# roeiherz/CanonicalSg2Im

Hardware: NVIDIA B200
Metric: scene_graphs_per_sec_gcn_layout_fwd_bwd (higher is better)
Workload: dtype bf16

## Files before the change

### canonicalsg2im_b200/csrc/gemm_tc.cu

```cuda
#include "common.cuh"
#include "internal.h"
#include <cuda.h>
#include <cuda_bf16.h>
#include <cuda_fp16.h>
#include <stdlib.h>
#include <string.h>

namespace {

constexpr int BLOCK_M = 128;
constexpr int BLOCK_K = 64;
constexpr int MAX_STAGES = 8;
constexpr int A_STAGE_BYTES = BLOCK_M * BLOCK_K * 2;
constexpr int GATHER_WARPS = 4;
constexpr int ACC_STRIDE = 256;
constexpr int SUB_N = 32;
constexpr int SUB_BYTES = 32 * SUB_N * 2;
constexpr int CHUNK_N = 64;
constexpr int CHUNK_BYTES = 32 * CHUNK_N * 2;
constexpr size_t SMEM_LIMIT = 232448;

enum { G_NONE = 0, G_A = 1, G_B = 2 };

struct TcParams {
  int M, N, K;
  int m_tiles, n_tiles, splits, kb_per_split, kb_total;
  int stages;
  int smem_epi;
  void* C;
  int ldc, out_f32;
  const float* bias;
  int relu;
  const float* rowscale;
  const __nv_bfloat16* mask_aux;
  int ld_aux;
  const int* g_sidx;
  const int* g_oidx;
  const int* g_pidx;
  int g_din, g_dp, g_rows;
  int debug;
  int a_f16, b_f16, c_f16;
  int tail_from, num_items;
};

__device__ __forceinline__ uint32_t smem_u32(const void* p) { return (uint32_t)__cvta_generic_to_shared(p); }

__device__ __forceinline__ void mbar_init(uint32_t bar, uint32_t count) {
  asm volatile("mbarrier.init.shared::cta.b64 [%0], %1;" ::"r"(bar), "r"(count));
}
__device__ __forceinline__ void mbar_arrive_expect_tx(uint32_t bar, uint32_t bytes) {
  asm volatile("mbarrier.arrive.expect_tx.shared::cta.b64 _, [%0], %1;" ::"r"(bar), "r"(bytes) : "memory");
}
// ... 115 lines not shown
      "%16, %17, %18, %19, %20, %21, %22, %23, %24, %25, %26, %27, %28, %29, %30, %31}, [%32];"
      : "=r"(r[0]), "=r"(r[1]), "=r"(r[2]), "=r"(r[3]), "=r"(r[4]), "=r"(r[5]), "=r"(r[6]), "=r"(r[7]),
        "=r"(r[8]), "=r"(r[9]), "=r"(r[10]), "=r"(r[11]), "=r"(r[12]), "=r"(r[13]), "=r"(r[14]), "=r"(r[15]),
        "=r"(r[16]), "=r"(r[17]), "=r"(r[18]), "=r"(r[19]), "=r"(r[20]), "=r"(r[21]), "=r"(r[22]), "=r"(r[23]),
        "=r"(r[24]), "=r"(r[25]), "=r"(r[26]), "=r"(r[27]), "=r"(r[28]), "=r"(r[29]), "=r"(r[30]), "=r"(r[31])
      : "r"(taddr)
      : "memory");
}
__device__ __forceinline__ void tmem_ld_wait() { asm volatile("tcgen05.wait::ld.sync.aligned;" ::: "memory"); }

__device__ __forceinline__ uint64_t make_desc(uint32_t saddr, uint32_t lbo_bytes, uint32_t sbo_bytes) {
  uint64_t d = 0;
  d |= (uint64_t)((saddr & 0x3FFFFu) >> 4);
  d |= (uint64_t)((lbo_bytes >> 4) & 0x3FFFu) << 16;
  d |= (uint64_t)((sbo_bytes >> 4) & 0x3FFFu) << 32;
  d |= (uint64_t)1 << 46;
  d |= (uint64_t)2 << 61;
  return d;
}
__host__ __device__ constexpr uint32_t make_idesc(int M, int N, bool a_mn, bool b_mn, bool a_f16 = false, bool b_f16 = false) {
  return (1u << 4) | ((a_f16 ? 0u : 1u) << 7) | ((b_f16 ? 0u : 1u) << 10) | ((a_mn ? 1u : 0u) << 15) |
         ((b_mn ? 1u : 0u) << 16) | ((uint32_t)(N >> 3) << 17) | ((uint32_t)(M >> 4) << 24);
}

struct __align__(8) Barriers {
  uint64_t full[MAX_STAGES];
  uint64_t empty[MAX_STAGES];
  uint64_t tmem_full[2];
  uint64_t tmem_empty[2];
  uint32_t tmem_base;
};

struct SmemPlan {
  uint32_t b, c, bias, bars, total;
};
__host__ __device__ inline SmemPlan smem_plan(int BN, int b_rows, int stages, bool smem_epi, int mt, int epw, bool sub32) {
  SmemPlan s;
  (void)BN;
  s.b = (uint32_t)stages * mt * A_STAGE_BYTES;
  s.c = s.b + (uint32_t)stages * b_rows * 128;
  s.bias = s.c + (smem_epi ? epw * (sub32 ? SUB_BYTES : CHUNK_BYTES) : 0);
  s.bars = s.bias + (smem_epi ? epw * (sub32 ? SUB_N : CHUNK_N) * 4 : 0);
  s.total = s.bars + (uint32_t)sizeof(Barriers);
  return s;
}

__device__ __forceinline__ uint32_t pack_bf16(float a, float b) {
  __nv_bfloat162 h = __floats2bfloat162_rn(a, b);
  return *reinterpret_cast<uint32_t*>(&h);
}
__device__ __forceinline__ uint32_t pack16(float a, float b, bool f16) {
  if (!f16) return pack_bf16(a, b);
  __half2 h = __floats2half2_rn(fminf(fmaxf(a, -65504.f), 65504.f), fminf(fmaxf(b, -65504.f), 65504.f));
  return *reinterpret_cast<uint32_t*>(&h);
}
__device__ __forceinline__ bool bf16_pos(uint32_t h) { return h != 0 && h < 0x8000u; }

template <int BN, bool MN, int GATHER, int CG, int MT, int EPW, bool SUB32>
__global__ void __launch_bounds__(64 + EPW * 32 + (GATHER != G_NONE ? GATHER_WARPS * 32 : 0), 1)
gemm_tc_kernel(const __grid_constant__ CUtensorMap tmA, const __grid_constant__ CUtensorMap tmB,
               const __grid_constant__ CUtensorMap tmP, const TcParams p) {
  extern __shared__ __align__(1024) uint8_t smem_raw[];
  const uint32_t base = smem_u32(smem_raw);
  uint8_t* base_ptr = smem_raw;
  if ((base & 1023u) != 0u) {
    if (threadIdx.x == 0) printf("csg gemm_tc: dynamic shared memory is not 1024-byte aligned\n");
    __trap();
  }
  static_assert(CG == 1 || !MN, "CTA pairs are implemented for the K-major kernels");
  static_assert(MT == 1 || (MN && GATHER == G_B && CG == 1 && MT * BN <= 512), "MT > 1: gathered-B MN-major kernels only");
  static_assert(EPW == 8 || EPW == 16, "epilogue warps: 2 or 4 per TMEM lane quarter");
  constexpr int EPI_WARPS = EPW;
  constexpr int FIRST_GATHER_WARP = 2 + EPW;
  constexpr int NSUB = EPW / 4;
  constexpr int A_STAGE = MT * A_STAGE_BYTES;
  constexpr int B_ROWS = BN / CG;
  constexpr int B_STAGE = B_ROWS * BLOCK_K * 2;
  constexpr int TILE_M = BLOCK_M * CG * MT;
  const uint32_t cta_rank = CG == 2 ? cluster_ctarank() : 0u;
  const int worker = CG == 2 ? (int)(blockIdx.x >> 1) : (int)blockIdx.x;
  const int nworkers = CG == 2 ? (int)(gridDim.x >> 1) : (int)gridDim.x;
  const bool has_aux = GATHER == G_NONE && p.mask_aux != nullptr;
  const SmemPlan plan = smem_plan(BN, B_ROWS, p.stages, p.smem_epi != 0, MT, EPW, SUB32);
  const uint32_t sA = base, sB = base + plan.b;
  Barriers* bars = reinterpret_cast<Barriers*>(base_ptr + plan.bars);
  const int warp = threadIdx.x >> 5, lane = threadIdx.x & 31;
  const int num_tiles = p.num_items;
  const int STAGES = p.stages;

  if (warp == 1 && lane == 0) {
    for (int s = 0; s < STAGES; ++s) {
      mbar_init(smem_u32(&bars->full[s]), 1);
      mbar_init(smem_u32(&bars->empty[s]), 1);
    }
    for (int s = 0; s < 2; ++s) {
      mbar_init(smem_u32(&bars->tmem_full[s]), 1);
      mbar_init(smem_u32(&bars->tmem_empty[s]), EPI_WARPS * CG);
    }
    asm volatile("fence.mbarrier_init.release.cluster;" ::: "memory");
  }
  if (warp == 0 && lane == 0) {
    tma_prefetch_desc(&tmA);
    tma_prefetch_desc(&tmB);
    if (GATHER != G_NONE) tma_prefetch_desc(&tmP);
  }
  if (warp == 2) {
    if (CG == 2) { tmem_alloc_pair(smem_u32(&bars->tmem_base), 512); tmem_relinquish_pair(); }
    else { tmem_alloc(smem_u32(&bars->tmem_base), 512); tmem_relinquish(); }
  }
  tc_fence_before();
  if (CG == 2) cluster_sync_all(); else __syncthreads();
  tc_fence_after();
  asm volatile("griddepcontrol.wait;" ::: "memory");
  const uint32_t tmem_base = bars->tmem_base;
  auto leader = [&](const uint64_t* bar) -> uint32_t { return CG == 2 ? mapa(smem_u32(bar), 0u) : smem_u32(bar); };

// ... 174 lines not shown
              uint64_t ad, bd;
              if (!MN) {
                ad = make_desc(a_base + k * 32, 16, 1024);
                bd = make_desc(b_base + k * 32, 16, 1024);
              } else {
                ad = make_desc(a_base + mi * A_STAGE_BYTES + k * 2048, 8192, 1024);
                bd = make_desc(b_base + k * 2048, 8192, 1024);
              }
              if (p.debug & 2) continue;
              if (CG == 2) umma_bf16_pair(d_tmem, ad, bd, idesc, (kb > kb0 || k > 0) ? 1u : 0u);
              else umma_bf16(d_tmem + mi * BN, ad, bd, idesc, (kb > kb0 || k > 0) ? 1u : 0u);
            }
          }
          if (CG == 2) {
            umma_commit_pair(smem_u32(&bars->empty[stage]));
            if (kb == kb1 - 1) umma_commit_pair(smem_u32(&bars->tmem_full[as]));
          } else {
            umma_commit(smem_u32(&bars->empty[stage]));
            if (kb == kb1 - 1) umma_commit(smem_u32(&bars->tmem_full[as]));
          }
          if (++stage == STAGES) { stage = 0; phase ^= 1; }
        }
        if (kb1 <= kb0) {
          if (CG == 2) umma_commit_pair(smem_u32(&bars->tmem_full[as])); else umma_commit(smem_u32(&bars->tmem_full[as]));
        }
      }
    }
  } else if (warp < FIRST_GATHER_WARP) {
    const int q = warp & 3;
    const int ew = warp - 2;
    const int sub = ew >> 2;
    int it = 0;
    if (!MN && p.smem_epi) {
      if constexpr (SUB32) {
      const uint32_t sC = base + plan.c + ew * SUB_BYTES;
      float* sbias = reinterpret_cast<float*>(base_ptr + plan.bias) + ew * SUB_N;
      const uint32_t sw = ((uint32_t)lane >> 1) & 3u;
      const uint32_t row_off = (uint32_t)lane * (SUB_N * 2);
      const int crow = lane >> 2, cpiece = lane & 3;
      __nv_bfloat16* Cb = reinterpret_cast<__nv_bfloat16*>(p.C);
      const bool cf16 = p.c_f16 != 0;
      for (int tile = worker; tile < num_tiles; tile += nworkers, ++it) {
        int mt, nt, sp, n0, nw;
        decode(tile, mt, nt, sp, n0, nw);
        const int as = it & 1, aphase = (it >> 1) & 1;
        const int row0 = mt * TILE_M + (int)cta_rank * BLOCK_M + q * 32;
        const int row = row0 + lane;
        const int ncols = min(nw, p.N - n0);
        const int nsb = (ncols + SUB_N - 1) / SUB_N;
        const bool warp_rows = row0 < p.M;
        const float rs = (p.rowscale && row < p.M) ? __ldg(p.rowscale + row) : 1.f;
        mbar_wait(smem_u32(&bars->tmem_full[as]), aphase);
        tc_fence_after();
        const uint32_t t_row = tmem_base + ((uint32_t)(q * 32) << 16) + as * ACC_STRIDE;
        const int my_last = nsb > sub ? ((nsb - 1 - sub) / NSUB) * NSUB + sub : -1;
        if ((p.debug & 4) || my_last < 0) {
          tc_fence_before();
          __syncwarp();
          if (lane == 0) { if (CG == 2) mbar_arrive_cluster(leader(&bars->tmem_empty[as])); else mbar_arrive(smem_u32(&bars->tmem_empty[as])); }
          continue;
        }
#pragma unroll 1
        for (int c = sub; c < nsb; c += NSUB) {
          const int col0 = n0 + c * SUB_N;
          const float bv = p.bias ? __ldg(p.bias + col0 + lane) : 0.f;
          uint32_t r[32];
          tmem_ld32(t_row + c * SUB_N, r);
          const int col = col0 + cpiece * 8;
          uint4 ax[4];
          if (has_aux && warp_rows) {
#pragma unroll
            for (int i = 0; i < 4; ++i) {
              const int rr = row0 + i * 8 + crow;
              ax[i] = rr < p.M ? __ldg(reinterpret_cast<const uint4*>(p.mask_aux + (size_t)rr * p.ld_aux + col))
                               : make_uint4(0u, 0u, 0u, 0u);
            }
          }
          tmem_ld_wait();
          if (c == my_last) {
            tc_fence_before();
            __syncwarp();
            if (lane == 0) { if (CG == 2) mbar_arrive_cluster(leader(&bars->tmem_empty[as])); else mbar_arrive(smem_u32(&bars->tmem_empty[as])); }
          }
          if (warp_rows) {
            float v[32];
#pragma unroll
            for (int j = 0; j < 32; ++j) v[j] = __uint_as_float(r[j]);
            if (p.bias) {
              sbias[lane] = bv;
              __syncwarp();
#pragma unroll
              for (int j = 0; j < 32; j += 4) {
                const float4 b = *reinterpret_cast<const float4*>(sbias + j);
                v[j] += b.x; v[j + 1] += b.y; v[j + 2] += b.z; v[j + 3] += b.w;
              }
            }
            if (p.relu) {
#pragma unroll
              for (int j = 0; j < 32; ++j) v[j] = fmaxf(v[j], 0.f);
            }
            if (p.rowscale) {
#pragma unroll
              for (int j = 0; j < 32; ++j) v[j] *= rs;
            }
#pragma unroll
            for (int j4 = 0; j4 < 4; ++j4) {
              const uint32_t off = row_off + ((((uint32_t)j4) ^ sw) << 4);
              const uint32_t u0 = pack16(v[j4 * 8], v[j4 * 8 + 1], cf16), u1 = pack16(v[j4 * 8 + 2], v[j4 * 8 + 3], cf16);
              const uint32_t u2 = pack16(v[j4 * 8 + 4], v[j4 * 8 + 5], cf16), u3 = pack16(v[j4 * 8 + 6], v[j4 * 8 + 7], cf16);
              asm volatile("st.shared.v4.u32 [%0], {%1, %2, %3, %4};" ::"r"(sC + off), "r"(u0), "r"(u1), "r"(u2), "r"(u3) : "memory");
            }
            __syncwarp();
#pragma unroll
            for (int i = 0; i < 4; ++i) {
              const int rl = i * 8 + crow;
              uint4 o;
              asm volatile("ld.shared.v4.u32 {%0, %1, %2, %3}, [%4];" : "=r"(o.x), "=r"(o.y), "=r"(o.z), "=r"(o.w)
                           : "r"(sC + (uint32_t)rl * (SUB_N * 2) + ((uint32_t)(cpiece ^ ((rl >> 1) & 3)) << 4)));
              if (has_aux) {
                const uint32_t a[4] = {ax[i].x, ax[i].y, ax[i].z, ax[i].w};
                uint32_t w[4] = {o.x, o.y, o.z, o.w};
#pragma unroll
                for (int e = 0; e < 4; ++e) {
                  if (!bf16_pos(a[e] & 0xFFFFu)) w[e] &= 0xFFFF0000u;
                  if (!bf16_pos(a[e] >> 16)) w[e] &= 0x0000FFFFu;
                }
                o = make_uint4(w[0], w[1], w[2], w[3]);
              }
              if (row0 + rl < p.M)
                *reinterpret_cast<uint4*>(Cb + (size_t)(row0 + rl) * p.ldc + col) = o;
            }
            __syncwarp();
          }
        }
      }
      } else {
      const uint32_t sC = base + plan.c + ew * CHUNK_BYTES;
      float* sbias = reinterpret_cast<float*>(base_ptr + plan.bias) + ew * CHUNK_N;
      const uint32_t sw = (uint32_t)(lane & 7) << 4;
      const uint32_t row_off = (uint32_t)lane * 128;
      const int crow = lane >> 3, cpiece = lane & 7;
      __nv_bfloat16* Cb = reinterpret_cast<__nv_bfloat16*>(p.C);
      const bool cf16 = p.c_f16 != 0;
      auto load_mask = [&](uint4 (&ax)[8], int row0, int col) {
#pragma unroll
        for (int i = 0; i < 8; ++i) {
          const int r = row0 + i * 4 + crow;
          ax[i] = (r < p.M && col < p.N) ? __ldg(reinterpret_cast<const uint4*>(p.mask_aux + (size_t)r * p.ld_aux + col))
                                         : make_uint4(0u, 0u, 0u, 0u);
        }
      };
      for (int tile = worker; tile < num_tiles; tile += nworkers, ++it) {
        int mt, nt, sp, n0, nw;
        decode(tile, mt, nt, sp, n0, nw);
        const int as = it & 1, aphase = (it >> 1) & 1;
        const int row0 = mt * TILE_M + (int)cta_rank * BLOCK_M + q * 32;
        const int row = row0 + lane;
        const int ncols = min(nw, p.N - n0);
        const int nchunks = (ncols + CHUNK_N - 1) / CHUNK_N;
        const bool warp_rows = row0 < p.M;
        const float rs = (p.rowscale && row < p.M) ? __ldg(p.rowscale + row) : 1.f;
        mbar_wait(smem_u32(&bars->tmem_full[as]), aphase);
        tc_fence_after();
        const uint32_t t_row = tmem_base + ((uint32_t)(q * 32) << 16) + as * ACC_STRIDE;
        const int my_last = nchunks > sub ? ((nchunks - 1 - sub) / NSUB) * NSUB + sub : -1;
        if ((p.debug & 4) || my_last < 0) {
          tc_fence_before();
          __syncwarp();
          if (lane == 0) { if (CG == 2) mbar_arrive_cluster(leader(&bars->tmem_empty[as])); else mbar_arrive(smem_u32(&bars->tmem_empty[as])); }
          continue;
        }
#pragma unroll 1
        for (int c = sub; c < nchunks; c += NSUB) {
          const int bc = n0 + c * CHUNK_N + lane;
          const float bv0 = (p.bias && bc < p.N) ? __ldg(p.bias + bc) : 0.f;
          const float bv1 = (p.bias && bc + 32 < p.N) ? __ldg(p.bias + bc + 32) : 0.f;
          uint32_t r0[32], r1[32];
          tmem_ld32(t_row + c * CHUNK_N, r0);
          tmem_ld32(t_row + c * CHUNK_N + 32, r1);
          const int col = n0 + c * CHUNK_N + cpiece * 8;
          uint4 ax[8];
          if (has_aux && warp_rows) load_mask(ax, row0, col);
          tmem_ld_wait();
          if (c == my_last) {
            tc_fence_before();
            __syncwarp();
            if (lane == 0) { if (CG == 2) mbar_arrive_cluster(leader(&bars->tmem_empty[as])); else mbar_arrive(smem_u32(&bars->tmem_empty[as])); }
          }
          if (warp_rows) {
            if (p.bias) {
              sbias[lane] = bv0; sbias[lane + 32] = bv1;
              __syncwarp();
            }
#pragma unroll
            for (int h = 0; h < 2; ++h) {
              float v[32];
#pragma unroll
              for (int j = 0; j < 32; ++j) v[j] = __uint_as_float(h ? r1[j] : r0[j]);
              if (p.bias) {
#pragma unroll
                for (int j = 0; j < 32; j += 4) {
                  float4 b = *reinterpret_cast<const float4*>(sbias + h * 32 + j);
                  v[j] += b.x; v[j + 1] += b.y; v[j + 2] += b.z; v[j + 3] += b.w;
                }
              }
              if (p.relu) {
#pragma unroll
                for (int j = 0; j < 32; ++j) v[j] = fmaxf(v[j], 0.f);
              }
              if (p.rowscale) {
#pragma unroll
                for (int j = 0; j < 32; ++j) v[j] *= rs;
              }
#pragma unroll
              for (int j4 = 0; j4 < 4; ++j4) {
                const uint32_t off = row_off + ((((uint32_t)(h * 4 + j4)) << 4) ^ sw);
                const uint32_t u0 = pack16(v[j4 * 8], v[j4 * 8 + 1], cf16), u1 = pack16(v[j4 * 8 + 2], v[j4 * 8 + 3], cf16);
                const uint32_t u2 = pack16(v[j4 * 8 + 4], v[j4 * 8 + 5], cf16), u3 = pack16(v[j4 * 8 + 6], v[j4 * 8 + 7], cf16);
                asm volatile("st.shared.v4.u32 [%0], {%1, %2, %3, %4};" ::"r"(sC + off), "r"(u0), "r"(u1), "r"(u2), "r"(u3) : "memory");
              }
            }
            __syncwarp();
#pragma unroll
            for (int i = 0; i < 8; ++i) {
              const int rl = i * 4 + crow;
              uint4 o;
              asm volatile("ld.shared.v4.u32 {%0, %1, %2, %3}, [%4];" : "=r"(o.x), "=r"(o.y), "=r"(o.z), "=r"(o.w)
                           : "r"(sC + (uint32_t)rl * 128 + ((uint32_t)(cpiece ^ (rl & 7)) << 4)));
              if (has_aux) {
                const uint32_t a[4] = {ax[i].x, ax[i].y, ax[i].z, ax[i].w};
                uint32_t w[4] = {o.x, o.y, o.z, o.w};
#pragma unroll
                for (int e = 0; e < 4; ++e) {
                  if (!bf16_pos(a[e] & 0xFFFFu)) w[e] &= 0xFFFF0000u;
                  if (!bf16_pos(a[e] >> 16)) w[e] &= 0x0000FFFFu;
                }
                o = make_uint4(w[0], w[1], w[2], w[3]);
              }
              if (row0 + rl < p.M && col < p.N)
                *reinterpret_cast<uint4*>(Cb + (size_t)(row0 + rl) * p.ldc + col) = o;
            }
            __syncwarp();
          }
        }
      }
      }
    } else {
      for (int tile = worker; tile < num_tiles; tile += nworkers, ++it) {
        int mt, nt, sp, n0, nw;
        decode(tile, mt, nt, sp, n0, nw);
        const int as = it & 1, aphase = (it >> 1) & 1;
        mbar_wait(smem_u32(&bars->tmem_full[as]), aphase);
        tc_fence_after();
#pragma unroll 1
        for (int ci = sub; ci < MT * (BN / 32); ci += NSUB) {
          const int mi = ci / (BN / 32), c = ci % (BN / 32);
          const int row = mt * TILE_M + (int)cta_rank * BLOCK_M + mi * BLOCK_M + q * 32 + lane;
          const bool rowok = row < p.M;
          const float rs = (p.rowscale && rowok) ? p.rowscale[row] : 1.f;
          const uint32_t t_row = tmem_base + ((uint32_t)(q * 32) << 16) + as * ACC_STRIDE + mi * BN;
          uint32_t r[32];
          tmem_ld32(t_row + c * 32, r);
          tmem_ld_wait();
          const int col = nt * BN + c * 32;
          if (rowok && col < p.N) {
            float v[32];
#pragma unroll
            for (int j = 0; j < 32; ++j) v[j] = __uint_as_float(r[j]);
            if (p.splits == 1) {
              if (p.bias) {
#pragma unroll
                for (int j = 0; j < 32; j += 4) {
                  float4 b = __ldg(reinterpret_cast<const float4*>(p.bias + col + j));
                  v[j] += b.x; v[j + 1] += b.y; v[j + 2] += b.z; v[j + 3] += b.w;
                }
              }
              if (p.relu) {
#pragma unroll
// ... 52 lines not shown

EncodeTiledFn get_encode() {
  static EncodeTiledFn fn = nullptr;
  if (!fn) {
    void* ptr = nullptr;
    cudaDriverEntryPointQueryResult q;
    if (cudaGetDriverEntryPoint("cuTensorMapEncodeTiled", &ptr, cudaEnableDefault, &q) == cudaSuccess &&
        q == cudaDriverEntryPointSuccess)
      fn = reinterpret_cast<EncodeTiledFn>(ptr);
  }
  return fn;
}

int make_map(CUtensorMap* map, const void* ptr, uint64_t inner, uint64_t outer, uint64_t row_bytes, uint32_t box_outer) {
  EncodeTiledFn enc = get_encode();
  CSG_REQUIRE(enc != nullptr, "gemm_tc: cuTensorMapEncodeTiled is not available from the driver");
  CSG_REQUIRE((reinterpret_cast<uintptr_t>(ptr) & 15) == 0 && (row_bytes & 15) == 0,
              "gemm_tc: operand pointer / pitch must be 16-byte aligned");
  cuuint64_t dims[2] = {inner, outer};
  cuuint64_t strides[1] = {row_bytes};
  cuuint32_t box[2] = {64, box_outer};
  cuuint32_t estr[2] = {1, 1};
  CUresult r = enc(map, CU_TENSOR_MAP_DATA_TYPE_BFLOAT16, 2, const_cast<void*>(ptr), dims, strides, box, estr,
                   CU_TENSOR_MAP_INTERLEAVE_NONE, CU_TENSOR_MAP_SWIZZLE_128B, CU_TENSOR_MAP_L2_PROMOTION_L2_256B,
                   CU_TENSOR_MAP_FLOAT_OOB_FILL_NONE);
  CSG_REQUIRE(r == CUDA_SUCCESS, "gemm_tc: cuTensorMapEncodeTiled failed (%d)", (int)r);
  return 0;
}

struct Maps {
  CUtensorMap a, b, p;
};

template <int BN, bool MN, int GATHER, int CG, int MT = 1, int EPW = 8, bool SUB32 = false>
int launch(const Maps& m, const TcParams& p, cudaStream_t stream) {
  const size_t smem = smem_plan(BN, BN / CG, p.stages, p.smem_epi != 0, MT, EPW, SUB32).total;
  CSG_REQUIRE(smem <= SMEM_LIMIT, "gemm_tc: shared-memory plan of %zu bytes exceeds the limit", smem);
  static bool configured = false;
  if (!configured) {
    CSG_CUDA(cudaFuncSetAttribute(gemm_tc_kernel<BN, MN, GATHER, CG, MT, EPW, SUB32>, cudaFuncAttributeMaxDynamicSharedMemorySize, (int)SMEM_LIMIT));
    configured = true;
  }
  const int tiles = p.m_tiles * p.n_tiles * p.splits;
  const int nthreads = 64 + EPW * 32 + (GATHER != G_NONE ? GATHER_WARPS * 32 : 0);
  if (CG == 1) {
    const int grid = tiles < csg_num_sms() ? tiles : csg_num_sms();
    cudaLaunchConfig_t cfg;
    memset(&cfg, 0, sizeof(cfg));
    cfg.gridDim = dim3(grid);
    cfg.blockDim = dim3(nthreads);
    cfg.dynamicSmemBytes = smem;
    cfg.stream = stream;
    cudaLaunchAttribute attr[1];
    attr[0].id = cudaLaunchAttributeProgrammaticStreamSerialization;
    attr[0].val.programmaticStreamSerializationAllowed = 1;
    cfg.attrs = attr; cfg.numAttrs = 1;
    CSG_CUDA(cudaLaunchKernelEx(&cfg, gemm_tc_kernel<BN, MN, GATHER, CG, MT, EPW, SUB32>, m.a, m.b, m.p, p));
  } else {
    const int pairs = csg_num_sms() / 2;
    cudaLaunchConfig_t cfg;
    memset(&cfg, 0, sizeof(cfg));
    cfg.gridDim = dim3(2 * (tiles < pairs ? tiles : pairs));
    cfg.blockDim = dim3(nthreads);
    cfg.dynamicSmemBytes = smem;
    cfg.stream = stream;
    cudaLaunchAttribute attr[2];
    attr[0].id = cudaLaunchAttributeClusterDimension;
    attr[0].val.clusterDim.x = 2; attr[0].val.clusterDim.y = 1; attr[0].val.clusterDim.z = 1;
    attr[1].id = cudaLaunchAttributeProgrammaticStreamSerialization;
    attr[1].val.programmaticStreamSerializationAllowed = 1;
    cfg.attrs = attr; cfg.numAttrs = 2;
    CSG_CUDA(cudaLaunchKernelEx(&cfg, gemm_tc_kernel<BN, MN, GATHER, CG, MT, EPW, SUB32>, m.a, m.b, m.p, p));
  }
  CSG_CHECK_LAUNCH("csg_gemm_bf16");
  return 0;
}

template <bool MN, int GATHER, int CG, int EPW = 8, bool SUB32 = false>
int launch_bn(int BN, const Maps& m, const TcParams& p, cudaStream_t stream) {
  switch (BN) {
    case 64: return launch<64, MN, GATHER, CG, 1, EPW, SUB32>(m, p, stream);
    case 128: return launch<128, MN, GATHER, CG, 1, EPW, SUB32>(m, p, stream);
    case 192: return launch<192, MN, GATHER, CG, 1, EPW, SUB32>(m, p, stream);
    case 256: return launch<256, MN, GATHER, CG, 1, EPW, SUB32>(m, p, stream);
  }
  csg_set_error("gemm_tc: unsupported BLOCK_N %d", BN);
  return 1;
}

int g_pair_mode = -1;

int kmajor_pick_bn(int M, int N) {
  int bn = N > 128 ? 256 : (N > 64 ? 128 : 64);
  const int m_tiles = csg_div_up(M, BLOCK_M);
  while (bn > 64 && m_tiles * csg_div_up(N, bn) < csg_num_sms()) bn >>= 1;
  return bn;
}

int pick_bn(int N) {
  if (N % 256 == 0) return 256;
  if (N % 192 == 0) return 192;
  if (N % 128 == 0) return 128;
  if (N >= 256) return 256;
  if (N > 128) return 192 >= N ? 192 : 256;
  if (N > 64) return 128;
  return 64;
}

void mn_split_plan(int M, int N, int K, int BN, int& kb_per_split, int& nsplits, int mt = 1) {
  const int tiles = csg_div_up(M, BLOCK_M * mt) * csg_div_up(N, BN);
  const int kb_total = csg_div_up(K, BLOCK_K);
  int splits = csg_num_sms() / tiles;
  if (splits < 1) splits = 1;
  if (splits > 64) splits = 64;
  if (splits > kb_total) splits = kb_total;
  kb_per_split = csg_div_up(kb_total, splits);
  nsplits = csg_div_up(kb_total, kb_per_split);
// ... 35 lines not shown
                                      mask_aux, ld_aux, g_obj, g_pred, g_sidx, g_oidx, g_din, g_dp, g_ldp, g_nobj, g_pidx, g_npred,
                                      formats, workspace, workspace_bytes, stream, &job)) return rc;
  return job.parts > 0 ? csg_reduce_multi(&job, 1, stream) : 0;
}

int csg_gemm_bf16_deferred(int mn_major, int gather, int M, int N, int K,
                           const void* A, int lda, const void* B, int ldb, void* C, int ldc, int out_f32,
                           const float* bias, int relu, const float* rowscale, const void* mask_aux, int ld_aux,
                           const void* g_obj, const void* g_pred, const int* g_sidx, const int* g_oidx,
                           int g_din, int g_dp, int g_ldp, int g_nobj, const int* g_pidx, int g_npred, int formats,
                           void* workspace, size_t workspace_bytes, cudaStream_t stream, CsgReduceJob* job) {
  job->parts = 0; job->n = 0; job->partial = nullptr; job->out = nullptr; job->stride = 0; job->lanes = 1;
  job->op = CSG_RED_SUM; job->aux = nullptr; job->ncols = 0; job->ldo = 0;
  if (M == 0 || N == 0) return 0;
  if (K == 0 && mn_major && out_f32 && M > 0 && N > 0) {
    CSG_CUDA(cudaMemset2DAsync(C, (size_t)ldc * 4, 0, (size_t)N * 4, M, stream));
    return 0;
  }
  CSG_REQUIRE(M > 0 && N > 0 && K > 0, "gemm_bf16: bad sizes M=%d N=%d K=%d", M, N, K);
  CsgProfScope prof(CSG_PROF_GEMM_BF16, 2.0 * M * N * K, stream);
  CSG_REQUIRE(N % 32 == 0, "gemm_bf16: N=%d must be a multiple of 32", N);
  CSG_REQUIRE((ldc % 8) == 0 || out_f32, "gemm_bf16: bf16 ldc must be a multiple of 8");
  CSG_REQUIRE(!out_f32 || (ldc % 4) == 0, "gemm_bf16: fp32 ldc must be a multiple of 4");
  TcParams p;
  p.M = M; p.N = N; p.K = K;
  p.C = C; p.ldc = ldc; p.out_f32 = out_f32;
  p.bias = bias; p.relu = relu; p.rowscale = rowscale;
  p.mask_aux = reinterpret_cast<const __nv_bfloat16*>(mask_aux); p.ld_aux = ld_aux;
  p.g_sidx = g_sidx; p.g_oidx = g_oidx; p.g_din = g_din; p.g_dp = g_dp;
  p.g_pidx = gather ? g_pidx : nullptr;
  CSG_REQUIRE(!p.g_pidx || g_npred > 0, "gemm_bf16: g_pidx needs the row count of the predicate table");
  p.g_rows = mn_major ? K : M;
  p.a_f16 = formats & 1; p.b_f16 = (formats >> 1) & 1; p.c_f16 = (formats >> 2) & 1;
  { const char* dbg = getenv("CSG_GEMM_DEBUG"); p.debug = dbg ? atoi(dbg) : 0; }
  if (gather) {
    CSG_REQUIRE(g_obj && g_pred && g_sidx && g_oidx && g_nobj > 0, "gemm_bf16: gather sources missing");
    CSG_REQUIRE(g_din % 64 == 0 && g_dp % 64 == 0 && g_ldp % 8 == 0, "gemm_bf16: gather dims must be multiples of 64");
    CSG_REQUIRE((gather == 1 && !mn_major && K == 2 * g_din + g_dp) || (gather == 2 && mn_major && N == 2 * g_din + g_dp),
                "gemm_bf16: gather mode / shape mismatch");
  }
  if (p.mask_aux) CSG_REQUIRE(ld_aux % 8 == 0, "gemm_bf16: ld_aux must be a multiple of 8");
  CSG_REQUIRE(!(gather && mask_aux), "gemm_bf16: the gathered GEMMs take no ReLU mask");
  const int BN = mn_major ? mn_pick_bn(M, N, gather) : kmajor_pick_bn(M, N);
  const int MT = (mn_major && mn_gather_mt4(M, N, gather)) ? GB_MT : 1;
  const bool pair = !mn_major && (BN % 32 == 0) && csg_num_sms() >= 2 &&
                    (g_pair_mode == 1 || (g_pair_mode < 0 && M >= 2 * BLOCK_M * csg_num_sms() && K >= 1024));
  const int CG = pair ? 2 : 1;
  const int epw = 8;
  bool sub32 = !mn_major && gather == 1;
  { const char* e = getenv("CSG_GEMM_EPI");
    if (e && !mn_major) sub32 = !strcmp(e, "8x32"); }
  p.m_tiles = csg_div_up(M, BLOCK_M * CG * MT);
  p.n_tiles = csg_div_up(N, BN);
  p.kb_total = csg_div_up(K, BLOCK_K);
  p.splits = 1;
  p.kb_per_split = p.kb_total;
  Maps maps;
  memset(&maps, 0, sizeof(maps));
  void* out = C;
  p.smem_epi = 0;
  p.stages = 4;
  if (!mn_major) {
    CSG_REQUIRE(K % 8 == 0, "gemm_bf16: K=%d must be a multiple of 8", K);
    if (gather == 1) {
      if (int rc = make_map(&maps.a, g_obj, g_din, g_nobj, (uint64_t)g_din * 2, 1)) return rc;
      if (p.g_pidx) { if (int rc = make_map(&maps.p, g_pred, g_dp, g_npred, (uint64_t)g_ldp * 2, 1)) return rc; }
      else if (int rc = make_map(&maps.p, g_pred, g_dp, M, (uint64_t)g_ldp * 2, BLOCK_M)) return rc;
    } else {
      if (int rc = make_map(&maps.a, A, K, M, (uint64_t)lda * 2, BLOCK_M)) return rc;
    }
    if (int rc = make_map(&maps.b, B, K, N, (uint64_t)ldb * 2, BN / CG)) return rc;
    p.smem_epi = (!out_f32 && (reinterpret_cast<uintptr_t>(C) & 15) == 0 &&
                  (!mask_aux || (reinterpret_cast<uintptr_t>(mask_aux) & 15) == 0)) ? 1 : 0;
    int best_s = 0;
    for (int st = (pair ? 6 : 5); st >= 2 && !best_s; --st)
      if (smem_plan(BN, BN / CG, st, p.smem_epi != 0, 1, epw, sub32).total <= SMEM_LIMIT) best_s = st;
    { const char* e = getenv("CSG_GEMM_STAGES"); if (e && atoi(e) >= 3 && atoi(e) < best_s) best_s = atoi(e); }
    CSG_REQUIRE(best_s > 0, "gemm_bf16: no shared-memory plan fits BN=%d", BN);
    p.stages = best_s;
  } else {
    CSG_REQUIRE(out_f32, "gemm_bf16: MN-major (weight-gradient) GEMMs write fp32");
    CSG_REQUIRE(!bias && !relu && !rowscale && !mask_aux, "gemm_bf16: MN-major GEMMs have no epilogue");
    mn_split_plan(M, N, K, BN, p.kb_per_split, p.splits, MT);
    if (p.splits > 1) {
      CSG_REQUIRE(ldc == N, "gemm_bf16: split-K output must be contiguous");
      CSG_REQUIRE(workspace && workspace_bytes >= (size_t)p.splits * M * N * sizeof(float), "gemm_bf16: workspace too small");
      p.C = workspace;
    }
    if (int rc = make_map(&maps.a, A, M, K, (uint64_t)lda * 2, 64)) return rc;
    if (gather == 2) {
      if (int rc = make_map(&maps.b, g_obj, g_din, g_nobj, (uint64_t)g_din * 2, 1)) return rc;
      if (p.g_pidx) { if (int rc = make_map(&maps.p, g_pred, g_dp, g_npred, (uint64_t)g_ldp * 2, 1)) return rc; }
      else if (int rc = make_map(&maps.p, g_pred, g_dp, K, (uint64_t)g_ldp * 2, 64)) return rc;
    } else {
      if (int rc = make_map(&maps.b, B, N, K, (uint64_t)ldb * 2, 64)) return rc;
    }
    p.stages = 5;
    while (p.stages > 2 && smem_plan(BN, BN, p.stages, false, MT, 8, false).total > SMEM_LIMIT) --p.stages;
    CSG_REQUIRE(MT == 1 || p.m_tiles * p.n_tiles * p.splits <= csg_num_sms(),
                "gemm_bf16: the multi-accumulator weight-gradient kernel needs one work item per CTA");
  }
  p.tail_from = -1;
  p.num_items = p.m_tiles * p.n_tiles * p.splits;
  {
    const char* e = getenv("CSG_GEMM_TAIL_SPLIT");
    const int T = p.m_tiles * p.n_tiles, W = pair ? csg_num_sms() / 2 : csg_num_sms();
    if (!(e && e[0] == '0') && !mn_major && p.smem_epi && p.splits == 1 && N % BN == 0 && BN >= 128 && T > W) {
      const int rem = T % W;
      if (rem > 0 && 2 * rem <= W) { p.tail_from = T - rem; p.num_items = T + rem; }
    }
  }
  int rc;
  if (!mn_major && pair)
    rc = gather == 1 ? (sub32 ? launch_bn<false, G_A, 2, 8, true>(BN, maps, p, stream) : launch_bn<false, G_A, 2>(BN, maps, p, stream))
                     : (sub32 ? launch_bn<false, G_NONE, 2, 8, true>(BN, maps, p, stream) : launch_bn<false, G_NONE, 2>(BN, maps, p, stream));
  else if (!mn_major)
    rc = gather == 1 ? (sub32 ? launch_bn<false, G_A, 1, 8, true>(BN, maps, p, stream) : launch_bn<false, G_A, 1>(BN, maps, p, stream))
                     : (sub32 ? launch_bn<false, G_NONE, 1, 8, true>(BN, maps, p, stream) : launch_bn<false, G_NONE, 1>(BN, maps, p, stream));
  else if (MT == GB_MT) rc = launch<128, true, G_B, 1, GB_MT>(maps, p, stream);
  else rc = gather == 2 ? launch_bn<true, G_B, 1>(BN, maps, p, stream) : launch_bn<true, G_NONE, 1>(BN, maps, p, stream);
  if (rc) return rc;
  if (p.splits > 1) {
    CSG_REQUIRE((long long)M * N < (1ll << 31), "gemm_bf16: split-K output too large");
    job->partial = reinterpret_cast<const float*>(p.C);
    job->out = reinterpret_cast<float*>(out);
    job->n = M * N; job->parts = p.splits; job->stride = (long long)M * N;
  }
  return 0;
}
```

Before: 29320.

## Write GEMM epilogue directly to global with 256-bit stores, drop smem staging

Replaces the shared-memory transpose-staged epilogue (and the 32-column variant) with per-thread row stores using 256-bit st.global.v8 and matching 256-bit mask loads, freeing the C staging buffer in shared memory. It also caches getenv lookups in statics and makes the kernel attribute setup per-device. This removes the smem round-trip and extra syncs and may let more pipeline stages fit, at the cost of uncoalesced per-row global writes (each lane writes a different row) and stricter 32-byte alignment requirements for the fast path.

```diff
diff --git a/canonicalsg2im_b200/csrc/gemm_tc.cu b/canonicalsg2im_b200/csrc/gemm_tc.cu
--- a/canonicalsg2im_b200/csrc/gemm_tc.cu
+++ b/canonicalsg2im_b200/csrc/gemm_tc.cu
@@ -14,10 +14,7 @@
 constexpr int A_STAGE_BYTES = BLOCK_M * BLOCK_K * 2;
 constexpr int GATHER_WARPS = 4;
 constexpr int ACC_STRIDE = 256;
-constexpr int SUB_N = 32;
-constexpr int SUB_BYTES = 32 * SUB_N * 2;
 constexpr int CHUNK_N = 64;
-constexpr int CHUNK_BYTES = 32 * CHUNK_N * 2;
 constexpr size_t SMEM_LIMIT = 232448;
 
 enum { G_NONE = 0, G_A = 1, G_B = 2 };
@@ -199,15 +196,14 @@
 };
 
 struct SmemPlan {
-  uint32_t b, c, bias, bars, total;
+  uint32_t b, bias, bars, total;
 };
-__host__ __device__ inline SmemPlan smem_plan(int BN, int b_rows, int stages, bool smem_epi, int mt, int epw, bool sub32) {
+__host__ __device__ inline SmemPlan smem_plan(int BN, int b_rows, int stages, bool smem_epi, int mt, int epw) {
   SmemPlan s;
   (void)BN;
   s.b = (uint32_t)stages * mt * A_STAGE_BYTES;
-  s.c = s.b + (uint32_t)stages * b_rows * 128;
-  s.bias = s.c + (smem_epi ? epw * (sub32 ? SUB_BYTES : CHUNK_BYTES) : 0);
-  s.bars = s.bias + (smem_epi ? epw * (sub32 ? SUB_N : CHUNK_N) * 4 : 0);
+  s.bias = s.b + (uint32_t)stages * b_rows * 128;
+  s.bars = s.bias + (smem_epi ? epw * CHUNK_N * 4 : 0);
   s.total = s.bars + (uint32_t)sizeof(Barriers);
   return s;
 }
@@ -223,7 +219,7 @@
 }
 __device__ __forceinline__ bool bf16_pos(uint32_t h) { return h != 0 && h < 0x8000u; }
 
-template <int BN, bool MN, int GATHER, int CG, int MT, int EPW, bool SUB32>
+template <int BN, bool MN, int GATHER, int CG, int MT, int EPW>
 __global__ void __launch_bounds__(64 + EPW * 32 + (GATHER != G_NONE ? GATHER_WARPS * 32 : 0), 1)
 gemm_tc_kernel(const __grid_constant__ CUtensorMap tmA, const __grid_constant__ CUtensorMap tmB,
                const __grid_constant__ CUtensorMap tmP, const TcParams p) {
@@ -248,7 +244,7 @@
   const int worker = CG == 2 ? (int)(blockIdx.x >> 1) : (int)blockIdx.x;
   const int nworkers = CG == 2 ? (int)(gridDim.x >> 1) : (int)gridDim.x;
   const bool has_aux = GATHER == G_NONE && p.mask_aux != nullptr;
-  const SmemPlan plan = smem_plan(BN, B_ROWS, p.stages, p.smem_epi != 0, MT, EPW, SUB32);
+  const SmemPlan plan = smem_plan(BN, B_ROWS, p.stages, p.smem_epi != 0, MT, EPW);
   const uint32_t sA = base, sB = base + plan.b;
   Barriers* bars = reinterpret_cast<Barriers*>(base_ptr + plan.bars);
   const int warp = threadIdx.x >> 5, lane = threadIdx.x & 31;
@@ -489,12 +485,7 @@
     const int sub = ew >> 2;
     int it = 0;
     if (!MN && p.smem_epi) {
-      if constexpr (SUB32) {
-      const uint32_t sC = base + plan.c + ew * SUB_BYTES;
-      float* sbias = reinterpret_cast<float*>(base_ptr + plan.bias) + ew * SUB_N;
-      const uint32_t sw = ((uint32_t)lane >> 1) & 3u;
-      const uint32_t row_off = (uint32_t)lane * (SUB_N * 2);
-      const int crow = lane >> 2, cpiece = lane & 3;
+      float* sbias = reinterpret_cast<float*>(base_ptr + plan.bias) + ew * CHUNK_N;
       __nv_bfloat16* Cb = reinterpret_cast<__nv_bfloat16*>(p.C);
       const bool cf16 = p.c_f16 != 0;
       for (int tile = worker; tile < num_tiles; tile += nworkers, ++it) {
@@ -503,120 +494,11 @@
         const int as = it & 1, aphase = (it >> 1) & 1;
         const int row0 = mt * TILE_M + (int)cta_rank * BLOCK_M + q * 32;
         const int row = row0 + lane;
-        const int ncols = min(nw, p.N - n0);
-        const int nsb = (ncols + SUB_N - 1) / SUB_N;
-        const bool warp_rows = row0 < p.M;
-        const float rs = (p.rowscale && row < p.M) ? __ldg(p.rowscale + row) : 1.f;
-        mbar_wait(smem_u32(&bars->tmem_full[as]), aphase);
-        tc_fence_after();
-        const uint32_t t_row = tmem_base + ((uint32_t)(q * 32) << 16) + as * ACC_STRIDE;
-        const int my_last = nsb > sub ? ((nsb - 1 - sub) / NSUB) * NSUB + sub : -1;
-        if ((p.debug & 4) || my_last < 0) {
-          tc_fence_before();
-          __syncwarp();
-          if (lane == 0) { if (CG == 2) mbar_arrive_cluster(leader(&bars->tmem_empty[as])); else mbar_arrive(smem_u32(&bars->tmem_empty[as])); }
-          continue;
-        }
-#pragma unroll 1
-        for (int c = sub; c < nsb; c += NSUB) {
-          const int col0 = n0 + c * SUB_N;
-          const float bv = p.bias ? __ldg(p.bias + col0 + lane) : 0.f;
-          uint32_t r[32];
-          tmem_ld32(t_row + c * SUB_N, r);
-          const int col = col0 + cpiece * 8;
-          uint4 ax[4];
-          if (has_aux && warp_rows) {
-#pragma unroll
-            for (int i = 0; i < 4; ++i) {
-              const int rr = row0 + i * 8 + crow;
-              ax[i] = rr < p.M ? __ldg(reinterpret_cast<const uint4*>(p.mask_aux + (size_t)rr * p.ld_aux + col))
-                               : make_uint4(0u, 0u, 0u, 0u);
-            }
-          }
-          tmem_ld_wait();
-          if (c == my_last) {
-            tc_fence_before();
-            __syncwarp();
-            if (lane == 0) { if (CG == 2) mbar_arrive_cluster(leader(&bars->tmem_empty[as])); else mbar_arrive(smem_u32(&bars->tmem_empty[as])); }
-          }
-          if (warp_rows) {
-            float v[32];
-#pragma unroll
-            for (int j = 0; j < 32; ++j) v[j] = __uint_as_float(r[j]);
-            if (p.bias) {
-              sbias[lane] = bv;
-              __syncwarp();
-#pragma unroll
-              for (int j = 0; j < 32; j += 4) {
-                const float4 b = *reinterpret_cast<const float4*>(sbias + j);
-                v[j] += b.x; v[j + 1] += b.y; v[j + 2] += b.z; v[j + 3] += b.w;
-              }
-            }
-            if (p.relu) {
-#pragma unroll
-              for (int j = 0; j < 32; ++j) v[j] = fmaxf(v[j], 0.f);
-            }
-            if (p.rowscale) {
-#pragma unroll
-              for (int j = 0; j < 32; ++j) v[j] *= rs;
-            }
-#pragma unroll
-            for (int j4 = 0; j4 < 4; ++j4) {
-              const uint32_t off = row_off + ((((uint32_t)j4) ^ sw) << 4);
-              const uint32_t u0 = pack16(v[j4 * 8], v[j4 * 8 + 1], cf16), u1 = pack16(v[j4 * 8 + 2], v[j4 * 8 + 3], cf16);
-              const uint32_t u2 = pack16(v[j4 * 8 + 4], v[j4 * 8 + 5], cf16), u3 = pack16(v[j4 * 8 + 6], v[j4 * 8 + 7], cf16);
-              asm volatile("st.shared.v4.u32 [%0], {%1, %2, %3, %4};" ::"r"(sC + off), "r"(u0), "r"(u1), "r"(u2), "r"(u3) : "memory");
-            }
-            __syncwarp();
-#pragma unroll
-            for (int i = 0; i < 4; ++i) {
-              const int rl = i * 8 + crow;
-              uint4 o;
-              asm volatile("ld.shared.v4.u32 {%0, %1, %2, %3}, [%4];" : "=r"(o.x), "=r"(o.y), "=r"(o.z), "=r"(o.w)
-                           : "r"(sC + (uint32_t)rl * (SUB_N * 2) + ((uint32_t)(cpiece ^ ((rl >> 1) & 3)) << 4)));
-              if (has_aux) {
-                const uint32_t a[4] = {ax[i].x, ax[i].y, ax[i].z, ax[i].w};
-                uint32_t w[4] = {o.x, o.y, o.z, o.w};
-#pragma unroll
-                for (int e = 0; e < 4; ++e) {
-                  if (!bf16_pos(a[e] & 0xFFFFu)) w[e] &= 0xFFFF0000u;
-                  if (!bf16_pos(a[e] >> 16)) w[e] &= 0x0000FFFFu;
-                }
-                o = make_uint4(w[0], w[1], w[2], w[3]);
-              }
-              if (row0 + rl < p.M)
-                *reinterpret_cast<uint4*>(Cb + (size_t)(row0 + rl) * p.ldc + col) = o;
-            }
-            __syncwarp();
-          }
-        }
-      }
-      } else {
-      const uint32_t sC = base + plan.c + ew * CHUNK_BYTES;
-      float* sbias = reinterpret_cast<float*>(base_ptr + plan.bias) + ew * CHUNK_N;
-      const uint32_t sw = (uint32_t)(lane & 7) << 4;
-      const uint32_t row_off = (uint32_t)lane * 128;
-      const int crow = lane >> 3, cpiece = lane & 7;
-      __nv_bfloat16* Cb = reinterpret_cast<__nv_bfloat16*>(p.C);
-      const bool cf16 = p.c_f16 != 0;
-      auto load_mask = [&](uint4 (&ax)[8], int row0, int col) {
-#pragma unroll
-        for (int i = 0; i < 8; ++i) {
-          const int r = row0 + i * 4 + crow;
-          ax[i] = (r < p.M && col < p.N) ? __ldg(reinterpret_cast<const uint4*>(p.mask_aux + (size_t)r * p.ld_aux + col))
-                                         : make_uint4(0u, 0u, 0u, 0u);
-        }
-      };
-      for (int tile = worker; tile < num_tiles; tile += nworkers, ++it) {
-        int mt, nt, sp, n0, nw;
-        decode(tile, mt, nt, sp, n0, nw);
-        const int as = it & 1, aphase = (it >> 1) & 1;
-        const int row0 = mt * TILE_M + (int)cta_rank * BLOCK_M + q * 32;
-        const int row = row0 + lane;
+        const bool rowok = row < p.M;
         const int ncols = min(nw, p.N - n0);
         const int nchunks = (ncols + CHUNK_N - 1) / CHUNK_N;
         const bool warp_rows = row0 < p.M;
-        const float rs = (p.rowscale && row < p.M) ? __ldg(p.rowscale + row) : 1.f;
+        const float rs = (p.rowscale && rowok) ? __ldg(p.rowscale + row) : 1.f;
         mbar_wait(smem_u32(&bars->tmem_full[as]), aphase);
         tc_fence_after();
         const uint32_t t_row = tmem_base + ((uint32_t)(q * 32) << 16) + as * ACC_STRIDE;
@@ -629,15 +511,28 @@
         }
 #pragma unroll 1
         for (int c = sub; c < nchunks; c += NSUB) {
-          const int bc = n0 + c * CHUNK_N + lane;
+          const int col0 = n0 + c * CHUNK_N;
+          const int bc = col0 + lane;
           const float bv0 = (p.bias && bc < p.N) ? __ldg(p.bias + bc) : 0.f;
           const float bv1 = (p.bias && bc + 32 < p.N) ? __ldg(p.bias + bc + 32) : 0.f;
           uint32_t r0[32], r1[32];
           tmem_ld32(t_row + c * CHUNK_N, r0);
           tmem_ld32(t_row + c * CHUNK_N + 32, r1);
-          const int col = n0 + c * CHUNK_N + cpiece * 8;
-          uint4 ax[8];
-          if (has_aux && warp_rows) load_mask(ax, row0, col);
+          uint32_t ax[4][8];
+          if (has_aux && rowok) {
+            const __nv_bfloat16* ap = p.mask_aux + (size_t)row * p.ld_aux + col0;
+#pragma unroll
+            for (int k = 0; k < 4; ++k) {
+              if (col0 + k * 16 < p.N)
+                asm volatile("ld.global.nc.v8.b32 {%0, %1, %2, %3, %4, %5, %6, %7}, [%8];"
+                             : "=r"(ax[k][0]), "=r"(ax[k][1]), "=r"(ax[k][2]), "=r"(ax[k][3]), "=r"(ax[k][4]),
+                               "=r"(ax[k][5]), "=r"(ax[k][6]), "=r"(ax[k][7])
+                             : "l"(ap + k * 16));
+              else
+#pragma unroll
+                for (int e = 0; e < 8; ++e) ax[k][e] = 0u;
+            }
+          }
           tmem_ld_wait();
           if (c == my_last) {
             tc_fence_before();
@@ -669,38 +564,30 @@
 #pragma unroll
                 for (int j = 0; j < 32; ++j) v[j] *= rs;
               }
-#pragma unroll
-              for (int j4 = 0; j4 < 4; ++j4) {
-                const uint32_t off = row_off + ((((uint32_t)(h * 4 + j4)) << 4) ^ sw);
-                const uint32_t u0 = pack16(v[j4 * 8], v[j4 * 8 + 1], cf16), u1 = pack16(v[j4 * 8 + 2], v[j4 * 8 + 3], cf16);
-                const uint32_t u2 = pack16(v[j4 * 8 + 4], v[j4 * 8 + 5], cf16), u3 = pack16(v[j4 * 8 + 6], v[j4 * 8 + 7], cf16);
-                asm volatile("st.shared.v4.u32 [%0], {%1, %2, %3, %4};" ::"r"(sC + off), "r"(u0), "r"(u1), "r"(u2), "r"(u3) : "memory");
+              const int col = col0 + h * 32;
+              if (rowok && col < p.N) {
+#pragma unroll
+                for (int s16 = 0; s16 < 2; ++s16) {
+                  uint32_t w[8];
+#pragma unroll
+                  for (int e = 0; e < 8; ++e) w[e] = pack16(v[s16 * 16 + 2 * e], v[s16 * 16 + 2 * e + 1], cf16);
+                  if (has_aux) {
+#pragma unroll
+                    for (int e = 0; e < 8; ++e) {
+                      const uint32_t a = ax[h * 2 + s16][e];
+                      if (!bf16_pos(a & 0xFFFFu)) w[e] &= 0xFFFF0000u;
+                      if (!bf16_pos(a >> 16)) w[e] &= 0x0000FFFFu;
+                    }
+                  }
+                  asm volatile("st.global.v8.b32 [%0], {%1, %2, %3, %4, %5, %6, %7, %8};"
+                               ::"l"(Cb + (size_t)row * p.ldc + col + s16 * 16), "r"(w[0]), "r"(w[1]), "r"(w[2]),
+                                 "r"(w[3]), "r"(w[4]), "r"(w[5]), "r"(w[6]), "r"(w[7]) : "memory");
+                }
               }
             }
             __syncwarp();
-#pragma unroll
-            for (int i = 0; i < 8; ++i) {
-              const int rl = i * 4 + crow;
-              uint4 o;
-              asm volatile("ld.shared.v4.u32 {%0, %1, %2, %3}, [%4];" : "=r"(o.x), "=r"(o.y), "=r"(o.z), "=r"(o.w)
-                           : "r"(sC + (uint32_t)rl * 128 + ((uint32_t)(cpiece ^ (rl & 7)) << 4)));
-              if (has_aux) {
-                const uint32_t a[4] = {ax[i].x, ax[i].y, ax[i].z, ax[i].w};
-                uint32_t w[4] = {o.x, o.y, o.z, o.w};
-#pragma unroll
-                for (int e = 0; e < 4; ++e) {
-                  if (!bf16_pos(a[e] & 0xFFFFu)) w[e] &= 0xFFFF0000u;
-                  if (!bf16_pos(a[e] >> 16)) w[e] &= 0x0000FFFFu;
-                }
-                o = make_uint4(w[0], w[1], w[2], w[3]);
-              }
-              if (row0 + rl < p.M && col < p.N)
-                *reinterpret_cast<uint4*>(Cb + (size_t)(row0 + rl) * p.ldc + col) = o;
-            }
-            __syncwarp();
           }
         }
-      }
       }
     } else {
       for (int tile = worker; tile < num_tiles; tile += nworkers, ++it) {
@@ -819,14 +706,24 @@
   CUtensorMap a, b, p;
 };
 
-template <int BN, bool MN, int GATHER, int CG, int MT = 1, int EPW = 8, bool SUB32 = false>
+constexpr int MAX_DEVICES = 64;
+
+int env_int(const char* name, int dflt) {
+  const char* e = getenv(name);
+  return e ? atoi(e) : dflt;
+}
+
+template <int BN, bool MN, int GATHER, int CG, int MT = 1, int EPW = 8>
 int launch(const Maps& m, const TcParams& p, cudaStream_t stream) {
-  const size_t smem = smem_plan(BN, BN / CG, p.stages, p.smem_epi != 0, MT, EPW, SUB32).total;
+  const size_t smem = smem_plan(BN, BN / CG, p.stages, p.smem_epi != 0, MT, EPW).total;
   CSG_REQUIRE(smem <= SMEM_LIMIT, "gemm_tc: shared-memory plan of %zu bytes exceeds the limit", smem);
-  static bool configured = false;
-  if (!configured) {
-    CSG_CUDA(cudaFuncSetAttribute(gemm_tc_kernel<BN, MN, GATHER, CG, MT, EPW, SUB32>, cudaFuncAttributeMaxDynamicSharedMemorySize, (int)SMEM_LIMIT));
-    configured = true;
+  static bool configured[MAX_DEVICES] = {};
+  int dev = 0;
+  CSG_CUDA(cudaGetDevice(&dev));
+  CSG_REQUIRE(dev < MAX_DEVICES, "gemm_tc: device %d out of range", dev);
+  if (!configured[dev]) {
+    CSG_CUDA(cudaFuncSetAttribute(gemm_tc_kernel<BN, MN, GATHER, CG, MT, EPW>, cudaFuncAttributeMaxDynamicSharedMemorySize, (int)SMEM_LIMIT));
+    configured[dev] = true;
   }
   const int tiles = p.m_tiles * p.n_tiles * p.splits;
   const int nthreads = 64 + EPW * 32 + (GATHER != G_NONE ? GATHER_WARPS * 32 : 0);
@@ -842,7 +739,7 @@
     attr[0].id = cudaLaunchAttributeProgrammaticStreamSerialization;
     attr[0].val.programmaticStreamSerializationAllowed = 1;
     cfg.attrs = attr; cfg.numAttrs = 1;
-    CSG_CUDA(cudaLaunchKernelEx(&cfg, gemm_tc_kernel<BN, MN, GATHER, CG, MT, EPW, SUB32>, m.a, m.b, m.p, p));
+    CSG_CUDA(cudaLaunchKernelEx(&cfg, gemm_tc_kernel<BN, MN, GATHER, CG, MT, EPW>, m.a, m.b, m.p, p));
   } else {
     const int pairs = csg_num_sms() / 2;
     cudaLaunchConfig_t cfg;
@@ -857,19 +754,19 @@
     attr[1].id = cudaLaunchAttributeProgrammaticStreamSerialization;
     attr[1].val.programmaticStreamSerializationAllowed = 1;
     cfg.attrs = attr; cfg.numAttrs = 2;
-    CSG_CUDA(cudaLaunchKernelEx(&cfg, gemm_tc_kernel<BN, MN, GATHER, CG, MT, EPW, SUB32>, m.a, m.b, m.p, p));
+    CSG_CUDA(cudaLaunchKernelEx(&cfg, gemm_tc_kernel<BN, MN, GATHER, CG, MT, EPW>, m.a, m.b, m.p, p));
   }
   CSG_CHECK_LAUNCH("csg_gemm_bf16");
   return 0;
 }
 
-template <bool MN, int GATHER, int CG, int EPW = 8, bool SUB32 = false>
+template <bool MN, int GATHER, int CG, int EPW = 8>
 int launch_bn(int BN, const Maps& m, const TcParams& p, cudaStream_t stream) {
   switch (BN) {
-    case 64: return launch<64, MN, GATHER, CG, 1, EPW, SUB32>(m, p, stream);
-    case 128: return launch<128, MN, GATHER, CG, 1, EPW, SUB32>(m, p, stream);
-    case 192: return launch<192, MN, GATHER, CG, 1, EPW, SUB32>(m, p, stream);
-    case 256: return launch<256, MN, GATHER, CG, 1, EPW, SUB32>(m, p, stream);
+    case 64: return launch<64, MN, GATHER, CG, 1, EPW>(m, p, stream);
+    case 128: return launch<128, MN, GATHER, CG, 1, EPW>(m, p, stream);
+    case 192: return launch<192, MN, GATHER, CG, 1, EPW>(m, p, stream);
+    case 256: return launch<256, MN, GATHER, CG, 1, EPW>(m, p, stream);
   }
   csg_set_error("gemm_tc: unsupported BLOCK_N %d", BN);
   return 1;
@@ -971,7 +868,8 @@
   CSG_REQUIRE(!p.g_pidx || g_npred > 0, "gemm_bf16: g_pidx needs the row count of the predicate table");
   p.g_rows = mn_major ? K : M;
   p.a_f16 = formats & 1; p.b_f16 = (formats >> 1) & 1; p.c_f16 = (formats >> 2) & 1;
-  { const char* dbg = getenv("CSG_GEMM_DEBUG"); p.debug = dbg ? atoi(dbg) : 0; }
+  static const int debug = env_int("CSG_GEMM_DEBUG", 0);
+  p.debug = debug;
   if (gather) {
     CSG_REQUIRE(g_obj && g_pred && g_sidx && g_oidx && g_nobj > 0, "gemm_bf16: gather sources missing");
     CSG_REQUIRE(g_din % 64 == 0 && g_dp % 64 == 0 && g_ldp % 8 == 0, "gemm_bf16: gather dims must be multiples of 64");
@@ -986,9 +884,6 @@
                     (g_pair_mode == 1 || (g_pair_mode < 0 && M >= 2 * BLOCK_M * csg_num_sms() && K >= 1024));
   const int CG = pair ? 2 : 1;
   const int epw = 8;
-  bool sub32 = !mn_major && gather == 1;
-  { const char* e = getenv("CSG_GEMM_EPI");
-    if (e && !mn_major) sub32 = !strcmp(e, "8x32"); }
   p.m_tiles = csg_div_up(M, BLOCK_M * CG * MT);
   p.n_tiles = csg_div_up(N, BN);
   p.kb_total = csg_div_up(K, BLOCK_K);
@@ -1009,12 +904,13 @@
       if (int rc = make_map(&maps.a, A, K, M, (uint64_t)lda * 2, BLOCK_M)) return rc;
     }
     if (int rc = make_map(&maps.b, B, K, N, (uint64_t)ldb * 2, BN / CG)) return rc;
-    p.smem_epi = (!out_f32 && (reinterpret_cast<uintptr_t>(C) & 15) == 0 &&
-                  (!mask_aux || (reinterpret_cast<uintptr_t>(mask_aux) & 15) == 0)) ? 1 : 0;
+    p.smem_epi = (!out_f32 && (reinterpret_cast<uintptr_t>(C) & 31) == 0 && ldc % 16 == 0 &&
+                  (!mask_aux || ((reinterpret_cast<uintptr_t>(mask_aux) & 31) == 0 && ld_aux % 16 == 0))) ? 1 : 0;
     int best_s = 0;
     for (int st = (pair ? 6 : 5); st >= 2 && !best_s; --st)
-      if (smem_plan(BN, BN / CG, st, p.smem_epi != 0, 1, epw, sub32).total <= SMEM_LIMIT) best_s = st;
-    { const char* e = getenv("CSG_GEMM_STAGES"); if (e && atoi(e) >= 3 && atoi(e) < best_s) best_s = atoi(e); }
+      if (smem_plan(BN, BN / CG, st, p.smem_epi != 0, 1, epw).total <= SMEM_LIMIT) best_s = st;
+    static const int stages_cap = env_int("CSG_GEMM_STAGES", 0);
+    if (stages_cap >= 3 && stages_cap < best_s) best_s = stages_cap;
     CSG_REQUIRE(best_s > 0, "gemm_bf16: no shared-memory plan fits BN=%d", BN);
     p.stages = best_s;
   } else {
@@ -1035,7 +931,7 @@
       if (int rc = make_map(&maps.b, B, N, K, (uint64_t)ldb * 2, 64)) return rc;
     }
     p.stages = 5;
-    while (p.stages > 2 && smem_plan(BN, BN, p.stages, false, MT, 8, false).total > SMEM_LIMIT) --p.stages;
+    while (p.stages > 2 && smem_plan(BN, BN, p.stages, false, MT, 8).total > SMEM_LIMIT) --p.stages;
     CSG_REQUIRE(MT == 1 || p.m_tiles * p.n_tiles * p.splits <= csg_num_sms(),
                 "gemm_bf16: the multi-accumulator weight-gradient kernel needs one work item per CTA");
   }
@@ -1051,11 +947,9 @@
   }
   int rc;
   if (!mn_major && pair)
-    rc = gather == 1 ? (sub32 ? launch_bn<false, G_A, 2, 8, true>(BN, maps, p, stream) : launch_bn<false, G_A, 2>(BN, maps, p, stream))
-                     : (sub32 ? launch_bn<false, G_NONE, 2, 8, true>(BN, maps, p, stream) : launch_bn<false, G_NONE, 2>(BN, maps, p, stream));
+    rc = gather == 1 ? launch_bn<false, G_A, 2>(BN, maps, p, stream) : launch_bn<false, G_NONE, 2>(BN, maps, p, stream);
   else if (!mn_major)
-    rc = gather == 1 ? (sub32 ? launch_bn<false, G_A, 1, 8, true>(BN, maps, p, stream) : launch_bn<false, G_A, 1>(BN, maps, p, stream))
-                     : (sub32 ? launch_bn<false, G_NONE, 1, 8, true>(BN, maps, p, stream) : launch_bn<false, G_NONE, 1>(BN, maps, p, stream));
+    rc = gather == 1 ? launch_bn<false, G_A, 1>(BN, maps, p, stream) : launch_bn<false, G_NONE, 1>(BN, maps, p, stream);
   else if (MT == GB_MT) rc = launch<128, true, G_B, 1, GB_MT>(maps, p, stream);
   else rc = gather == 2 ? launch_bn<true, G_B, 1>(BN, maps, p, stream) : launch_bn<true, G_NONE, 1>(BN, maps, p, stream);
   if (rc) return rc;
```

Result: no change. 29590, median of 6 (+0.9%).
